# sp-uhh/audio-visual-vad

Hardware: AMD Instinct MI355X
Metric: AV frame-pairs/sec (fwd+bwd) (higher is better)
Workload: dtype f32; 1 GPU; AV_net fused training step (WaveNet-W0 encoder + ResNet-18 trunk + concat + 2xLSTM1024 + FC, masked BCE, backward, RCCL all-reduce, fused Adam): BASELINE configs[3]/[4] per-GPU shard; per_gpu_frame_pairs=1024, global_frame_pairs=1024, sequences_per_gpu=64, parallelism=dp1, reserved_cus=0, reported_block=median

## Files before the change

### audio-visual-vad_amd/csrc/igemm.h

```cpp
#pragma once
#include "common.h"
#include <type_traits>

namespace igemm {

constexpr int BK = 32;

struct NoCtx {};

struct EpiStore {
  static constexpr bool PLAIN = true;
  float* C;
  long ldc;
  const float* bias;
  int mode;
  int cs = 1;
  double* stat = nullptr;
  __device__ __forceinline__ float* ptr(int m, int n) const { return C + (long)m * ldc + (long)n * cs; }
};
template <class Epi, class = void>
struct HasStat : std::false_type {};
template <class Epi>
struct HasStat<Epi, std::void_t<decltype(Epi::stat)>> : std::true_type {};

// ... 308 lines not shown
template <class Epi, class = void>
struct HasFinish : std::false_type {};
template <class Epi>
struct HasFinish<Epi, std::void_t<decltype(&Epi::finish4)>> : std::true_type {};

typedef __bf16 bf16x8 __attribute__((ext_vector_type(8)));
typedef __bf16 bf16x4 __attribute__((ext_vector_type(4)));
typedef float f32x4v __attribute__((ext_vector_type(4)));
constexpr int LDH = 40;

template <class Op, int BX, int NTH>
struct Stage {
  static constexpr int VEC = Op::VEC;
  static constexpr int NV = BX * BK / (NTH * VEC);
  static constexpr int LD = Op::KCONTIG ? BX + 1 : BX + 4;
  static constexpr int NCTX = (Op::KCONTIG || PerVec<Op>::value) ? NV : 1;
  static constexpr int TILE_F32 = BK * LD;
  static constexpr int TILE_BF = BX * LDH / 2;
  __device__ static __forceinline__ void coord(int t, int i, int& xl, int& kl) {
    if (Op::KCONTIG) {
      if (VEC == 4) { kl = (t & 7) * 4; xl = (t >> 3) + (NTH / 8) * i; }
      else { kl = t & 31; xl = (t >> 5) + (NTH / 32) * i; }
    } else {
      if (VEC == 4) { constexpr int Q = BX / 4; xl = (t % Q) * 4; kl = t / Q + (NTH / Q) * i; }
      else { xl = t % BX; kl = t / BX + (NTH / BX) * i; }
    }
  }
  __device__ static __forceinline__ void to_lds(float* S, int t, const float (&st0)[NV][VEC], const Op& op, unsigned okmask) {
    float st[NV][VEC];
#pragma unroll
    for (int i = 0; i < NV; ++i)
#pragma unroll
      for (int j = 0; j < VEC; ++j) {
        float v = st0[i][j];
        if constexpr (HasPost<Op>::value) v = op.post(v);
#ifdef AVVAD_ABL_NOSEL
        st[i][j] = v;
#else
        st[i][j] = ((okmask >> i) & 1u) ? v : 0.f;
#endif
      }
#pragma unroll
    for (int i = 0; i < NV; ++i) {
      int xl, kl;
      coord(t, i, xl, kl);
      if constexpr (Op::KCONTIG) {
#pragma unroll
        for (int j = 0; j < VEC; ++j) S[(kl + j) * LD + xl] = st[i][j];
      } else if constexpr (VEC == 4) {
        *reinterpret_cast<float4*>(S + kl * LD + xl) = make_float4(st[i][0], st[i][1], st[i][2], st[i][3]);
      } else {
        S[kl * LD + xl] = st[i][0];
      }
    }
  }
  __device__ static __forceinline__ void to_lds_bf(__bf16* S, int t, const float (&st0)[NV][VEC], const Op& op, unsigned okmask) {
#pragma unroll
    for (int i = 0; i < NV; ++i) {
      int xl, kl;
      coord(t, i, xl, kl);
      float st[VEC];
#pragma unroll
      for (int j = 0; j < VEC; ++j) {
        float v = st0[i][j];
        if constexpr (HasPost<Op>::value) v = op.post(v);
        st[j] = ((okmask >> i) & 1u) ? v : 0.f;
      }
      if (Op::KCONTIG) {
        if constexpr (VEC == 4) {
          const f32x4v f = {st[0], st[1], st[2], st[3]};
          *reinterpret_cast<bf16x4*>(S + xl * LDH + kl) = __builtin_convertvector(f, bf16x4);
        } else {
          S[xl * LDH + kl] = (__bf16)st[0];
        }
      } else {
#pragma unroll
        for (int j = 0; j < VEC; ++j) S[(xl + j) * LDH + kl] = (__bf16)st[j];
      }
    }
  }
};

template <int BM, int BN, bool DB, int NTH, class AOp, class BOp, class Epi, bool BF = false>
__global__ void __launch_bounds__(NTH, NTH == 512 ? 4 : ((DB || BM * BN < 128 * 128) ? 2 : 3))
    kernel(const AOp A, const BOp B, const Epi E, const int M, const int N, const int flags, const int ktiles,
           const int full_rounds, const int rem_tiles, const int kchunks, float* __restrict__ const slab) {
  const bool stagger = (flags & 1) != 0;
  typedef Stage<AOp, BM, NTH> SA;
  typedef Stage<BOp, BN, NTH> SB;
  constexpr int WGN = (BM == 256) ? 2 : NTH / 128;
  constexpr int WGM = NTH / 64 / WGN;
  constexpr int TM = BM / (32 * WGM), TN = BN / (32 * WGN);
  constexpr int TILE = BF ? SA::TILE_BF + SB::TILE_BF : BK * SA::LD + BK * SB::LD;
  constexpr int AOFF = BF ? SA::TILE_BF : BK * SA::LD;
  const int t_stage = threadIdx.x;
  __shared__ __attribute__((aligned(16))) float smem[(DB ? 2 : 1) * TILE];
  auto stage = [&](float* dst, const float (&ra)[SA::NV][SA::VEC], const float (&rb)[SB::NV][SB::VEC], unsigned ma, unsigned mb) {
    if constexpr (BF) {
      SA::to_lds_bf(reinterpret_cast<__bf16*>(dst), t_stage, ra, A, ma);
      SB::to_lds_bf(reinterpret_cast<__bf16*>(dst + AOFF), t_stage, rb, B, mb);
    } else {
      SA::to_lds(dst, t_stage, ra, A, ma);
      SB::to_lds(dst + AOFF, t_stage, rb, B, mb);
    }
  };

  const int t = threadIdx.x;
  const int lane = t & 63, wave = t >> 6;
  const int li = lane & 31, lh = lane >> 5;
  const int wm = wave / WGN, wn = wave % WGN;
  const int ntn = (N + BN - 1) / BN;

#ifdef AVVAD_PROF
  if (t == 0 && blockIdx.x < 2048) {
    g_prof_blk[2 * blockIdx.x] = __builtin_amdgcn_s_memrealtime();
    g_prof_clk[blockIdx.x] = __builtin_amdgcn_s_memtime();
    g_prof_hw[blockIdx.x] = ((unsigned long long)__builtin_amdgcn_s_getreg((3 << 11) | (0 << 6) | 20) << 32) |
                            (unsigned)__builtin_amdgcn_s_getreg((31 << 11) | (0 << 6) | 4);
  }
#endif
  const long G = gridDim.x;
  const long g = xcd_remap(blockIdx.x, gridDim.x);
  long rem_iters = (long)rem_tiles * ktiles;
  if constexpr (HasSched<Epi>::value) rem_iters = E.sched.total();
  long it = g * rem_iters / G;
  const long it_end = (g + 1) * rem_iters / G;
  const long ntiles_all = (long)((M + BM - 1) / BM) * ntn;
  int round = 0;
  long cell = g;

  for (;;) {
    int tile, kt0, kt1;
    int klen = ktiles;
    if (kchunks > 0) {
      if (cell >= (long)kchunks * ntiles_all) break;
      const int c = (int)(cell / ntiles_all);
      tile = (int)(cell - (long)c * ntiles_all);
      kt0 = (int)((long)c * ktiles / kchunks);
      kt1 = (int)((long)(c + 1) * ktiles / kchunks);
      cell += G;
      if (kt1 <= kt0) continue;
    } else if (round < full_rounds) {
      const long tl = (long)round * G + g;
      ++round;
      if (tl >= ntiles_all) continue;
      tile = (int)tl; kt0 = 0; kt1 = ktiles;
    } else if (it < it_end) {
      if constexpr (HasSched<Epi>::value) {
        E.sched.locate(it, tile, kt0, klen);
      } else {
        const long tr = it / ktiles;
        tile = (int)((long)full_rounds * G + tr);
        kt0 = (int)(it - tr * ktiles);
      }
      kt1 = (int)min((long)klen, kt0 + (it_end - it));
      it += kt1 - kt0;
    } else {
      break;
    }
    const int m0 = (tile / ntn) * BM, n0 = (tile % ntn) * BN;

    typename AOp::Ctx actx[SA::NCTX];
    typename BOp::Ctx bctx[SB::NCTX];
#pragma unroll
    for (int i = 0; i < SA::NCTX; ++i) {
      int xl, kl;
      SA::coord(t, i, xl, kl);
// ... 477 lines not shown

template <int BM, int BN, class AOp, class BOp, class Epi>
static inline int launch(const AOp& a, const BOp& b, const Epi& e_in, int M, int N, int K, int split_k_hint,
                         hipStream_t s, float* slab = nullptr, bool allow_bf16 = true, bool* finished = nullptr) {
  Epi e = e_in;
  if (M <= 0 || N <= 0 || K <= 0) return AVVAD_EINVAL;
  const int ktiles = (K + BK - 1) / BK;
  const long ntiles = (long)cdiv(M, BM) * cdiv(N, BN);
  const long iters = ntiles * ktiles;
  const AvvadTune& tn = avvad_tune();
  const int var = tn.igemm_variant;
  constexpr bool BIG = (BM == 128 && BN == 128);
  constexpr bool TALL = (BM == 256);
  const int variant = TALL ? 3 : (var >= 0 ? var : (BIG ? 2 : 1));
  int per_cu;
  if (variant == 3) per_cu = 2;
  else if (variant == 0) per_cu = BIG ? 2 : (BM * BN >= 128 * 64 ? 3 : 4);
  else if (variant == 1 || !BIG) per_cu = BIG ? 3 : (BM * BN >= 128 * 64 ? 4 : 6);
  else per_cu = 2;
  const int cus = (tn.max_cus > 0 && tn.max_cus < NUM_CU) ? tn.max_cus : NUM_CU;
  long G = (long)cus * per_cu;
  if (G * BM * BN > (long)SLAB_FLOATS) G = (long)(SLAB_FLOATS / ((size_t)BM * BN));
  const bool no_sk = !slab || tn.no_streamk == 1 || tn.no_streamk == 10 + e.mode ||
                     (double)ntiles * ktiles * (double)G >= 4.0e9;
  long full_rounds = ntiles / G, rem = ntiles - full_rounds * G;
  int kchunks = 0;
  if (split_k_hint > 1 && e.mode != 0 && ntiles <= G && tn.kmajor) {
    long best = -1;
    for (int r = 1; r <= 2; ++r) {
      long nc = r * G / ntiles;
      if (nc > ktiles) nc = ktiles;
      if (nc < 1) nc = 1;
      const long rr = (nc * ntiles + G - 1) / G;
      const long cost = rr * ((ktiles + nc - 1) / nc) + rr * 8;
      if (best < 0 || cost < best) { best = cost; kchunks = (int)nc; }
    }
    full_rounds = 0; rem = 0;
    if ((long)kchunks * ntiles < G) G = (long)kchunks * ntiles;
  } else {
    if (no_sk || rem * 10 >= G * 9) {
      if (rem > 0) ++full_rounds;
      rem = 0;
    }
    if (rem > 0 && full_rounds == 0) {
      const long cap = iters / 4 > 0 ? iters / 4 : 1;
      if (G > cap) G = cap;
    }
  }
  const int fr = (int)full_rounds, rt = (int)rem;
  const bool bf = allow_bf16 && tn.bf16;
  bool stat = false;
  if constexpr (std::is_same<Epi, EpiStore>::value) {
    stat = e.stat != nullptr;
    if (stat && (e.cs != 1 || (e.ldc & 3) || (N & 3) || (((uintptr_t)e.C) & 15) || kchunks > 0 || e.bias != nullptr)) return AVVAD_EINVAL;
  }
  if constexpr (HasFinish<Epi>::value) {
    e.active = (rt > 0 && kchunks == 0 && fr == 0 && (long)rt == ntiles) ? 1 : 0;
    if (finished) *finished = e.active != 0;
  } else if (finished) {
    *finished = false;
  }
  const int kflags = tn.stagger ? 1 : 0;
#define AVVAD_IGEMM_LAUNCH(DBV, NTHV)                                                                                       \
  do {                                                                                                                      \
    if (bf)                                                                                                                 \
      hipLaunchKernelGGL((kernel<BM, BN, DBV, NTHV, AOp, BOp, Epi, true>), dim3((int)G), dim3(NTHV), 0, s, a, b, e, M, N, kflags, \
                         ktiles, fr, rt, kchunks, slab);                                                                    \
    else                                                                                                                    \
      hipLaunchKernelGGL((kernel<BM, BN, DBV, NTHV, AOp, BOp, Epi, false>), dim3((int)G), dim3(NTHV), 0, s, a, b, e, M, N, kflags, \
                         ktiles, fr, rt, kchunks, slab);                                                                    \
  } while (0)
  if constexpr (TALL) {
    AVVAD_IGEMM_LAUNCH(false, 512);
  } else {
    if (variant == 0) AVVAD_IGEMM_LAUNCH(true, 256);
    else if (variant == 1 || !BIG) AVVAD_IGEMM_LAUNCH(false, 256);
    else AVVAD_IGEMM_LAUNCH(true, (BIG ? 512 : 256));
  }
#undef AVVAD_IGEMM_LAUNCH
  if (rt > 0 && kchunks == 0 && stat) {
    if constexpr (std::is_same<Epi, EpiStore>::value)
      hipLaunchKernelGGL((fixup_tile<BM, BN>), dim3(rt), dim3(256), 0, s, e, slab, M, N, ktiles, G, fr, rt, cdiv(N, BN));
  } else if (rt > 0 && kchunks == 0) {
    const int deep = tn.no_fixup1 > 1 ? tn.no_fixup1 : 6;
    if ((G + rt - 1) / rt <= deep && tn.no_fixup1 != 1)
      hipLaunchKernelGGL((fixup1<BM, BN, Epi>), dim3(rt * (BM * BN / 1024)), dim3(256), 0, s, e, slab, M, N, ktiles, G, fr, rt, cdiv(N, BN));
    else
      hipLaunchKernelGGL((fixup<BM, BN, Epi>), dim3(rt * (BM * BN / 256)), dim3(256), 0, s, e, slab, M, N, ktiles, G, fr, rt, cdiv(N, BN));
  }
  AVVAD_LAUNCH_CHECK();
  return AVVAD_OK;
}

template <class AOp, class BOp, class Epi>
static inline int launch_cls(const AOp& a, const BOp& b, const Epi& e, int Mp, int N, hipStream_t s, float* slab) {
  constexpr int BM = 128, BN = 128;
  if (Mp <= 0 || N <= 0 || !slab) return AVVAD_EINVAL;
  const AvvadTune& tn = avvad_tune();
  const long ntiles = (long)cdiv(Mp, BM) * cdiv(N, BN);
  const int cus = (tn.max_cus > 0 && tn.max_cus < NUM_CU) ? tn.max_cus : NUM_CU;
  long G = (long)cus * 2;
  if (G * BM * BN > (long)SLAB_FLOATS) G = (long)(SLAB_FLOATS / ((size_t)BM * BN));
  const long R = e.sched.total();
  if (R <= 0 || (double)R * (double)G >= 4.0e9) return AVVAD_EINVAL;
  if (G > R / 4) G = R / 4 > 0 ? R / 4 : 1;
  bool stat = false;
  if constexpr (HasStat<Epi>::value) {
    stat = e.stat != nullptr;
    if (stat && (e.cs != 1 || (e.ldc & 3) || (N & 3) || (((uintptr_t)e.C) & 15) || (e.W & 3))) return AVVAD_EINVAL;
  }
  hipLaunchKernelGGL((kernel<BM, BN, true, 512, AOp, BOp, Epi, false>), dim3((int)G), dim3(512), 0, s, a, b, e, Mp, N,
                     tn.stagger ? 1 : 0, 1, 0, (int)ntiles, 0, slab);
  if (stat) {
    if constexpr (HasStat<Epi>::value)
      hipLaunchKernelGGL((fixup_tile<BM, BN, Epi>), dim3((int)ntiles), dim3(256), 0, s, e, slab, Mp, N, 1, G, 0, (int)ntiles, cdiv(N, BN));
  } else if ((G + ntiles - 1) / ntiles <= 6) {
    hipLaunchKernelGGL((fixup1<BM, BN, Epi>), dim3((int)ntiles * (BM * BN / 1024)), dim3(256), 0, s, e, slab, Mp, N, 1, G, 0,
                       (int)ntiles, cdiv(N, BN));
  } else {
    hipLaunchKernelGGL((fixup<BM, BN, Epi>), dim3((int)ntiles * (BM * BN / 256)), dim3(256), 0, s, e, slab, Mp, N, 1, G, 0, (int)ntiles,
                       cdiv(N, BN));
  }
  AVVAD_LAUNCH_CHECK();
  return AVVAD_OK;
}

}
```

### audio-visual-vad_amd/csrc/trunk.hip

```cpp
#include "bgemm.h"
#include "conv64.h"

using convop::Geom;

namespace {

#include "bn_kernels.h"

constexpr int NCONV = AVVAD_TRUNK_NCONV;

struct ConvSpec {
  int cin, cout, ks, stride, pad;
  int stage;
  int role;
};

struct Plan {
  int N, H, W;
  int h[6], w[6];
  ConvSpec conv[NCONV];
  Geom geom[NCONV];
  size_t wf[NCONV], wd[NCONV];
  size_t wf16[NCONV], wd16[NCONV];
  size_t bn_scale, bn_shift, bn_mean, bn_invstd;
// ... 392 lines not shown
      const int r = i / W, c = i - r * W;
      img[(r + 3) * LDW + c + 3] = xn[i];
    }
    __syncthreads();
    const __amdgpu_buffer_rsrc_t rdy = brsrc(dy + (long)n * Ho * Wo * 64, Ho * Wo * 64 * 4);
    constexpr int RB = 4;
    float b0[RB][STEM_WH], b1[RB][STEM_WH];
    auto rowload = [&](int ho0, float (&b)[RB][STEM_WH]) {
#pragma unroll
      for (int rr = 0; rr < RB; ++rr)
#pragma unroll
        for (int sw = 0; sw < STEM_WH; ++sw)
          b[rr][sw] = bload(rdy, (sw < wh && ho0 + rr < Ho) ? voff : BUF_OOB, ((ho0 + rr) * Wo + 2 * sw) * 256);
    };
    auto rowmul = [&](int ho0, const float (&b)[RB][STEM_WH]) {
#pragma unroll
      for (int rr = 0; rr < RB; ++rr) {
        if (ho0 + rr >= Ho) break;
        const float* ap = img + abase + 2 * (ho0 + rr) * LDW;
#pragma unroll
        for (int sw = 0; sw < STEM_WH; ++sw)
          if (sw < wh) acc = mfma32(ap[4 * sw], b[rr][sw], acc);
      }
    };
    rowload(0, b0);
    for (int ho = 0; ho < Ho; ho += 2 * RB) {
      if (ho + RB < Ho) rowload(ho + RB, b1);
      __builtin_amdgcn_sched_barrier(0);
      rowmul(ho, b0);
      if (ho + RB >= Ho) break;
      if (ho + 2 * RB < Ho) rowload(ho + 2 * RB, b0);
      __builtin_amdgcn_sched_barrier(0);
      rowmul(ho + RB, b1);
    }
  }
  float* out = slab + (long)blockIdx.x * (49 * 64);
#pragma unroll
  for (int r = 0; r < 16; ++r) {
    const int t = mt * 32 + mfma32_row(r, lh);
    if (t < 49) out[t * 64 + nt * 32 + li] = acc[r];
  }
}
__global__ void __launch_bounds__(256) stem_wgrad_reduce(const float* __restrict__ slab, int nslab, float* __restrict__ pk) {
  __shared__ float sm[8][32];
  const int el = threadIdx.x & 31, grp = threadIdx.x >> 5;
  const int i = blockIdx.x * 32 + el;
  float s = 0.f;
#pragma unroll 4
  for (int b = grp; b < nslab; b += 8) s += slab[(long)b * (49 * 64) + i];
  sm[grp][el] = s;
  __syncthreads();
  if (grp != 0) return;
#pragma unroll
  for (int k = 1; k < 8; ++k) s += sm[k][el];
  pk[i] = s;
}

static inline bool fits_u30(long n) { return n >= 0 && n < (1L << 30); }
static inline bool taps_fit(const Geom& g) { return g.KS * g.KS <= 32; }
static inline bool fits_buf(long n_floats) { return n_floats >= 0 && n_floats < (1L << 29) - 64; }
static inline bool stem_kernel_ok(const Geom& g) {
  const int LDW = (g.W + 6) | 1;
  return g.C == 1 && g.KS == 7 && g.stride == 2 && g.pad == 3 && g.Co == 64 && (size_t)(g.H + 6) * LDW * sizeof(float) <= 48 * 1024 &&
         !avvad_tune().no_stem_kernel;
}
static inline bool stem_wgrad_ok(const Geom& g, bool slab) {
  return stem_kernel_ok(g) && (g.Wo & 1) == 0 && g.Wo <= 2 * STEM_WH && slab && (long)g.Ho * g.Wo * 64 * 4 < (1L << 31);
}
static inline long cls_tile_cap() {
  if (avvad_tune().cls_cap > 0) return avvad_tune().cls_cap;
  return 4L * ((avvad_tune().max_cus > 0 && avvad_tune().max_cus < 256) ? avvad_tune().max_cus : 256);
}
static inline bool cls_common(const Geom& g, bool slab) {
  return avvad_tune().bf16 == 0 && !avvad_tune().no_cls && slab && g.KS == 3 && g.pad == 1 && g.N >= 128 && g.C % 32 == 0 &&
         g.Co % 32 == 0 && g.Ho >= 2 && g.Wo >= 2 && avvad_tune().igemm_variant < 0 && !avvad_tune().no_buf &&
         avvad_tune().no_streamk == 0;
}
static inline bool conv_fwd_cls_ok(const Geom& g, bool slab) {
  if (!cls_common(g, slab) || g.Co % 4 || g.Co < 128) return false;
  const long tiles = (long)g.Ho * g.Wo * cdiv(g.N, 128) * cdiv(g.Co, 128);
  return tiles <= cls_tile_cap() &&
         fits_buf((long)g.N * g.H * g.W * g.C) && fits_buf(9L * g.C * g.Co);
}
static inline bool conv_dgrad_cls_ok(const Geom& g, bool slab) {
  if (!cls_common(g, slab) || (g.stride != 1 && (g.stride != 2 || avvad_tune().no_s2_cls)) || g.C % 4 || g.C < 128) return false;
  const long tiles = (long)g.H * g.W * cdiv(g.N, 128) * cdiv(g.C, 128);
  return tiles <= cls_tile_cap() &&
         fits_buf((long)g.N * g.Ho * g.Wo * g.Co) && fits_buf(9L * g.C * g.Co);
}
static inline bool conv_wgrad_tap_ok(const Geom& g, bool slab) {
  if (!cls_common(g, slab) || g.C % 128 || g.Co % 4 || g.Co < 128) return false;
  return 9L * (g.C / 128) * cdiv(g.Co, 128) <= cls_tile_cap() &&
         fits_buf((long)g.N * g.H * g.W * g.C) && fits_buf((long)g.N * g.Ho * g.Wo * g.Co);
}
static inline int conv64_cus() { return (avvad_tune().max_cus > 0 && avvad_tune().max_cus < 256) ? avvad_tune().max_cus : 256; }
static inline bool conv64_ok(const Geom& g, bool b16) {
  const long M = (long)g.N * g.H * g.W;
  return (b16 || avvad_tune().bf16 == 0) && !avvad_tune().no_conv64 && g.C == 64 && g.Co == 64 && g.KS == 3 && g.stride == 1 &&
         g.pad == 1 && g.Ho == g.H && g.Wo == g.W && M > 0 && fits_buf(M * 64) &&
         (unsigned long)(M + 64) * (unsigned long)(g.H * g.W) < 0x100000000ull;
}
static inline bool conv64_wgrad_ok(const Geom& g, bool slab) {
  return conv64_ok(g, false) && slab && g.W <= conv64::WG_MAXW && (size_t)conv64_cus() * conv64::WG_PART <= igemm::SLAB_FLOATS &&
         (long)g.N * g.H * g.W * 256 < (1L << 31);
}

static inline bool native_bf16() { return avvad_tune().bf16 == 1; }
static inline bool bf16_conv_ok(const Geom& g) {
  return g.C % 64 == 0 && g.Co % 64 == 0 && taps_fit(g) && fits_buf((long)g.N * g.H * g.W * g.C / 2) &&
         fits_buf((long)g.N * g.Ho * g.Wo * g.Co / 2) && fits_buf((long)g.KS * g.KS * g.C * g.Co / 2);
}
static inline bool cls16_common(const Geom& g, bool slab) {
  return !avvad_tune().no_cls && slab && g.KS == 3 && g.pad == 1 && g.N >= 128 && g.Ho >= 2 && g.Wo >= 2 && g.Ho * g.Wo <= 9 &&
         avvad_tune().no_streamk == 0;
}
static inline bool conv_fwd16_cls_ok(const Geom& g, bool slab) {
  if (!cls16_common(g, slab) || g.Co < 128) return false;
  return (long)g.Ho * g.Wo * cdiv(g.N, 128) * cdiv(g.Co, 128) <= cls_tile_cap();
}
static inline bool conv_dgrad16_cls_ok(const Geom& g, bool slab) {
  const bool form = g.stride == 1 ? cls16_common(g, slab)
                                  : g.stride == 2 && g.KS == 3 && g.pad == 1 && !avvad_tune().no_cls && !avvad_tune().no_s2_cls &&
                                        avvad_tune().no_streamk == 0 && slab && g.N >= 128;
  return form && g.C >= 128 && (long)g.H * g.W * cdiv(g.N, 128) * cdiv(g.C, 128) <= cls_tile_cap();
}
static inline bool conv_wgrad16_tap_ok(const Geom& g, bool slab) {
  return cls16_common(g, slab) && g.C % 128 == 0 && g.Co >= 128 && 9L * (g.C / 128) * cdiv(g.Co, 128) <= cls_tile_cap();
}

enum Form { STEM, CONV64, CLS, TAP, PARITY, ENGINE };
struct ConvForm {
  Form form;
  int rows, cols;
  bool buf;
  int chunks;
};
static ConvForm fwd_form(const Geom& g, bool b16, bool slab) {
  const long M = (long)g.N * g.Ho * g.Wo;
  const int cols = g.Co <= 64 ? 64 : 128;
  if (conv64_ok(g, b16)) return {CONV64, 0, 0, false, conv64::grid_for((long)g.N * g.H * g.W, conv64_cus())};
  if (b16 ? conv_fwd16_cls_ok(g, slab) : conv_fwd_cls_ok(g, slab)) return {CLS, 0, 0, false, g.Ho * g.Wo * cdiv(g.N, 128)};
  if (b16) return {ENGINE, 128, cols, true, cdiv(M, 128)};
  if (g.C == 1) return stem_kernel_ok(g) ? ConvForm{STEM, 0, 0, false, g.N} : ConvForm{ENGINE, 128, 64, false, 0};
  const int rows = g.Co <= 64 && !avvad_tune().no_tall ? 256 : 128;
  const bool buf = fits_buf((long)g.N * g.H * g.W * g.C) && fits_buf((long)g.KS * g.KS * g.C * g.Co) && !avvad_tune().no_buf;
  return {ENGINE, rows, cols, buf, cdiv(M, rows)};
}
static ConvForm dgrad_form(const Geom& g, bool b16, bool slab) {
  if (conv64_ok(g, b16)) return {CONV64};
  if (b16 ? conv_dgrad16_cls_ok(g, slab) : conv_dgrad_cls_ok(g, slab)) return {CLS};
  const int cols = g.C <= 64 ? 64 : 128;
  const bool buf = b16 || (fits_buf((long)g.N * g.Ho * g.Wo * g.Co) && fits_buf((long)g.KS * g.KS * g.C * g.Co) && !avvad_tune().no_buf);
  if (g.stride == 2) return {PARITY, 128, cols, buf};
  return {ENGINE, cols == 64 && !b16 && !avvad_tune().no_tall ? 256 : 128, cols, buf};
}
static ConvForm wgrad_form(const Geom& g, bool b16, bool slab) {
  const int cols = g.Co <= 64 ? 64 : 128;
  if (b16) return conv_wgrad16_tap_ok(g, slab) ? ConvForm{TAP} : ConvForm{ENGINE, 128, cols, true};
  if (conv64_wgrad_ok(g, slab)) return {CONV64};
  if (conv_wgrad_tap_ok(g, slab)) return {TAP};
  if (g.C == 1) return stem_wgrad_ok(g, slab) ? ConvForm{STEM} : ConvForm{ENGINE, 64, 64, false};
  const bool buf = fits_buf((long)g.N * g.H * g.W * g.C) && fits_buf((long)g.N * g.Ho * g.Wo * g.Co) && !avvad_tune().no_buf;
  return {ENGINE, 128, cols, buf};
}

static igemm::ClassSched fwd_sched(const Geom& g, int kc) {
  const int lsh = ((g.Ho - 1) * g.stride - g.pad + 2 > g.H - 1) ? 1 : 0, lsw = ((g.Wo - 1) * g.stride - g.pad + 2 > g.W - 1) ? 1 : 0;
  return igemm::ClassSched{g.Ho, g.Wo, cdiv(g.Co, 128), g.C / kc, cdiv(g.N, 128), 3, 1, lsh, 1, lsw};
}
static igemm::ClassSched dgrad_sched(const Geom& g, int kc) {
  igemm::ClassSched sc{g.H, g.W, cdiv(g.C, 128), g.Co / kc, cdiv(g.N, 128), 3, 1, 1, 1, 1};
  if (g.stride == 2) { sc.s2 = 1; sc.Hq = g.Ho; sc.Wq = g.Wo; }
  return sc;
}
template <class Gemm>
static int dgrad_parity(float* dx, const Geom& g, int accumulate, hipStream_t s, Gemm gemm) {
  const long n = (long)g.N * g.H * g.W * g.C;
  if (!accumulate) hipLaunchKernelGGL(zero_f32, dim3(ew_grid(n)), dim3(256), 0, s, dx, n);
  for (int ph = 0; ph < 2; ++ph)
    for (int pw = 0; pw < 2; ++pw) {
      convop::S2Class c;
      c.ph = ph; c.pw = pw;
      c.Hc = (g.H - ph + 1) / 2; c.Wc = (g.W - pw + 1) / 2;
      c.kh0 = (ph + g.pad) & 1; c.kw0 = (pw + g.pad) & 1;
      c.nkh = c.kh0 < g.KS ? (g.KS - c.kh0 + 1) / 2 : 0;
      c.nkw = c.kw0 < g.KS ? (g.KS - c.kw0 + 1) / 2 : 0;
      c.oh = (ph + g.pad - c.kh0) / 2; c.ow = (pw + g.pad - c.kw0) / 2;
      const int Mc = g.N * c.Hc * c.Wc, ntap = c.nkh * c.nkw;
      if (Mc <= 0 || ntap <= 0) continue;
      if (ntap > 4) return AVVAD_EINVAL;
      c.mg_ntap = convop::div_magic(ntap); c.mg_nkw = convop::div_magic(c.nkw);
      const convop::EpiS2 e{dx, g.C, nullptr, 1, 1, g.H, g.W, c.Hc, c.Wc, ph, pw, convop::div_magic(c.Hc * c.Wc), convop::div_magic(c.Wc)};
      if ((unsigned long)(Mc + 128) * (unsigned long)(c.Hc * c.Wc) >= 0x100000000ull) return AVVAD_EINVAL;
      if (const int rc = gemm(c, Mc, ntap, e)) return rc;
    }
  return AVVAD_OK;
}

static int conv64_launch(bool b16, bool flip, const float* x, const float* wpk, float* y, const Geom& g, int accumulate, hipStream_t s,
                         double* stat) {
  const int M = g.N * g.H * g.W;
  const int grid = conv64::grid_for(M, conv64_cus());
  const unsigned mg_hw = convop::div_magic((unsigned)(g.H * g.W)), mg_w = convop::div_magic((unsigned)g.W);
  auto k = b16 ? (flip ? conv64::kernel16<true> : conv64::kernel16<false>) : (flip ? conv64::kernel<true> : conv64::kernel<false>);
  hipLaunchKernelGGL(k, dim3(grid), dim3(conv64::NW * 64), 0, s, x, wpk, y, M, g.H, g.W, mg_hw, mg_w, accumulate, stat);
  AVVAD_LAUNCH_CHECK();
  return AVVAD_OK;
}
static int conv_fwd_cls(const float* x, const float* wf, float* y, const Geom& g, hipStream_t s, float* slab, double* stat) {
  const int MB = cdiv(g.N, 128), P = g.Ho * g.Wo;
  const igemm::ClassSched sc = fwd_sched(g, 32);
  const igemm::ClassRow cr{P, convop::div_magic(P)};
  convop::Im2colFwdCls a{x, g, g.N, cr, sc};
  convop::ColTapRowsCls b{wf, g.Co, g.Co, g.C, 3, 0, cr, sc};
  igemm::EpiCls e{y, (long)P * g.Co, nullptr, 0};
  e.stat = stat; e.W = g.Co; e.rows = g.N; e.cr = cr; e.sched = sc;
  return igemm::launch_cls(a, b, e, MB * P * 128, g.Co, s, slab);
}
static int conv_dgrad_cls(const float* dy, const float* wd, float* dx, const Geom& g, int accumulate, hipStream_t s, float* slab) {
  const int MB = cdiv(g.N, 128), P = g.H * g.W;
  const igemm::ClassSched sc = dgrad_sched(g, 32);
  const igemm::ClassRow cr{P, convop::div_magic(P)};
  convop::Im2colDgradCls a{dy, g, g.N, cr, sc};
  convop::ColTapRowsCls b{wd, g.C, g.C, g.Co, 3, 1, cr, sc};
  igemm::EpiCls e{dx, (long)P * g.C, nullptr, accumulate ? 1 : 0};
  e.W = g.C; e.rows = g.N; e.cr = cr; e.sched = sc;
  return igemm::launch_cls(a, b, e, MB * P * 128, g.C, s, slab);
}

template <bool BUF>
static int conv_fwd_t(const float* x, const float* wf, float* y, const Geom& g, const ConvForm& f, hipStream_t s, float* slab, double* stat) {
  const int M = g.N * g.Ho * g.Wo, K = g.KS * g.KS * g.C;
  igemm::EpiStore e{y, g.Co, nullptr, 0};
  if (g.C == 1) {
    igemm::ColPlain<4> b{wf, g.Co, g.Co, K, 0};
    convop::StemFwd a{x, g, M, K};
    return igemm::launch<128, 64>(a, b, e, M, g.Co, K, 1, s, slab);
  }
  e.stat = stat;
  if (g.C % 32 || g.Co % 4 || !taps_fit(g)) return AVVAD_EINVAL;
  if (!fits_u30((long)g.N * g.H * g.W * g.C) || !fits_u30((long)K * g.Co)) return AVVAD_EINVAL;
  const int T = g.KS * g.KS;
  convop::ColTapRows<BUF> b{wf, g.Co, g.Co, K, g.C, T, convop::div_magic(T)};
  convop::Im2colFwd<BUF> a{x, g, M, convop::tap_div(T, g.KS)};
  if (f.rows == 256) return igemm::launch<256, 64>(a, b, e, M, g.Co, K, 1, s, slab);
  if (f.cols == 64) return igemm::launch<128, 64>(a, b, e, M, g.Co, K, 1, s, slab);
  return igemm::launch<128, 128>(a, b, e, M, g.Co, K, 1, s, slab);
}
static int conv_fwd(const float* x, const float* wf, float* y, const Geom& g, hipStream_t s, float* slab, double* stat = nullptr) {
  const ConvForm f = fwd_form(g, false, slab);
  switch (f.form) {
    case STEM: {
      const int LDW = (g.W + 6) | 1;
      hipLaunchKernelGGL(stem_fwd_mfma, dim3(g.N), dim3(256), (size_t)(g.H + 6) * LDW * sizeof(float), s, x, wf, y, g.H, g.W, g.Ho, g.Wo,
                         LDW, stat);
      AVVAD_LAUNCH_CHECK();
      return AVVAD_OK;
    }
    case CONV64: return conv64_launch(false, false, x, wf, y, g, 0, s, stat);
    case CLS: return conv_fwd_cls(x, wf, y, g, s, slab, stat);
    default: return f.buf ? conv_fwd_t<true>(x, wf, y, g, f, s, slab, stat) : conv_fwd_t<false>(x, wf, y, g, f, s, slab, stat);
  }
}
template <bool BUF>
static int conv_dgrad_t(const float* dy, const float* wd, float* dx, const Geom& g, const ConvForm& f, int accumulate, hipStream_t s,
                        float* slab) {
  const int M = g.N * g.H * g.W, K = g.KS * g.KS * g.Co;
  if (g.Co % 32 || g.C % 4 || !taps_fit(g)) return AVVAD_EINVAL;
  if (!fits_u30((long)g.N * g.Ho * g.Wo * g.Co) || !fits_u30((long)K * g.C)) return AVVAD_EINVAL;
  if (f.form == PARITY)
    return dgrad_parity(dx, g, accumulate, s, [&](const convop::S2Class& c, int Mc, int ntap, const convop::EpiS2& e) {
      convop::Im2colDgradS2<BUF> a{dy, g, c, Mc};
      convop::ColSegRows<BUF> b{wd, g.C, g.C, ntap * g.Co, ntap, {0, 0, 0, 0}, convop::div_magic(ntap)};
      for (int ia = 0; ia < c.nkh; ++ia)
        for (int ib = 0; ib < c.nkw; ++ib) b.rowbase[ia * c.nkw + ib] = ((c.kh0 + 2 * ia) * g.KS + (c.kw0 + 2 * ib)) * g.Co;
      return f.cols == 64 ? igemm::launch<128, 64>(a, b, e, Mc, g.C, ntap * g.Co, 1, s, slab)
                          : igemm::launch<128, 128>(a, b, e, Mc, g.C, ntap * g.Co, 1, s, slab);
    });
  igemm::EpiStore e{dx, g.C, nullptr, accumulate ? 1 : 0};
  const int T = g.KS * g.KS;
  convop::ColTapRows<BUF> b{wd, g.C, g.C, K, g.Co, T, convop::div_magic(T)};
  convop::Im2colDgrad<BUF> a{dy, g, M, convop::tap_div(T, g.KS)};
  if (f.rows == 256) return igemm::launch<256, 64>(a, b, e, M, g.C, K, 1, s, slab);
  if (f.cols == 64) return igemm::launch<128, 64>(a, b, e, M, g.C, K, 1, s, slab);
  return igemm::launch<128, 128>(a, b, e, M, g.C, K, 1, s, slab);
}
static int conv_dgrad(const float* dy, const float* wd, float* dx, const Geom& g, int accumulate, hipStream_t s, float* slab) {
  const ConvForm f = dgrad_form(g, false, slab);
  switch (f.form) {
    case CONV64: return conv64_launch(false, true, dy, wd, dx, g, accumulate, s, nullptr);
    case CLS: return conv_dgrad_cls(dy, wd, dx, g, accumulate, s, slab);
    default: return f.buf ? conv_dgrad_t<true>(dy, wd, dx, g, f, accumulate, s, slab) : conv_dgrad_t<false>(dy, wd, dx, g, f, accumulate, s, slab);
  }
}
template <bool BUF>
static int conv_wgrad_t(const float* x, const float* dy, float* pk, const Geom& g, const ConvForm& f, hipStream_t s, float* slab) {
  const int M = g.KS * g.KS * g.C, K = g.N * g.Ho * g.Wo;
  igemm::ColPlain<4, BUF> b{dy, g.Co, g.Co, K, 0};
  const int ktiles = cdiv(K, igemm::BK);
  if (g.C == 1) {
    igemm::EpiStore e{pk, g.Co, nullptr, 0};
    convop::StemWgradX a{x, g, M, K};
    int split = 1024; if (split > ktiles) split = ktiles;
    return igemm::launch<64, 64>(a, b, e, M, g.Co, K, split, s, slab);
  }
  if (g.C % 32) return AVVAD_EINVAL;
  convop::EpiWgrad e{pk, g.Co, nullptr, 0, 1, g.C, g.KS * g.KS, convop::div_magic(g.KS * g.KS)};
  if ((unsigned long)(K + igemm::BK) * (unsigned long)(g.Ho * g.Wo) >= 0x100000000ull) return AVVAD_EINVAL;
  if (!fits_u30((long)g.N * g.H * g.W * g.C) || !fits_u30((long)K * g.Co)) return AVVAD_EINVAL;
  convop::WgradX<BUF> a{x, g, M, K, convop::div_magic(g.Ho * g.Wo), convop::div_magic(g.Wo)};
  const int nb = cdiv(M, 128) * cdiv(g.Co, f.cols);
  int split = cdiv(1024, nb); if (split > ktiles) split = ktiles;
  if (f.cols == 64) return igemm::launch<128, 64>(a, b, e, M, g.Co, K, split, s, slab);
  return igemm::launch<128, 128>(a, b, e, M, g.Co, K, split, s, slab);
}
static inline igemm::TapSched tap_sched(const Geom& g, int tiles_per_tap) {
  const int NP = cdiv(g.N, 128) * 128;
  const int lsh = ((g.Ho - 1) * g.stride - g.pad + 2 > g.H - 1) ? 1 : 0, lsw = ((g.Wo - 1) * g.stride - g.pad + 2 > g.W - 1) ? 1 : 0;
  return igemm::TapSched{g.Ho, g.Wo, tiles_per_tap, NP / 32, 3, 1, lsh, 1, lsw};
}
static int conv_wgrad_tap(const float* x, const float* dy, float* pk, const Geom& g, hipStream_t s, float* slab) {
  const int M = 9 * g.C;
  const igemm::TapSched sc = tap_sched(g, (g.C / 128) * cdiv(g.Co, 128));
  convop::WgradXTap a{x, g, M, g.C, g.N, convop::div_magic(g.C), sc};
  convop::ColDyTap b{dy, g, g.Co, g.C, g.N, sc};
  igemm::EpiTap e{pk, g.Co, nullptr, 0};
  e.Mrows = M; e.sched = sc;
  return igemm::launch_cls(a, b, e, M, g.Co, s, slab);
}
static int conv64_wgrad(const float* x, const float* dy, float* pk, const Geom& g, hipStream_t s, float* slab) {
  const int NR = g.N * g.H;
  const int grid = NR < conv64_cus() ? NR : conv64_cus();
  hipLaunchKernelGGL(conv64::wgrad_kernel, dim3(grid), dim3(conv64::WG_WAVES * 64), 0, s, x, dy, slab, NR, g.H, g.W,
                     convop::div_magic((unsigned)g.H));
  hipLaunchKernelGGL(conv64::wgrad_reduce, dim3(conv64::WG_PART / 256), dim3(256), 0, s, (const float*)slab, grid, pk);
  AVVAD_LAUNCH_CHECK();
  return AVVAD_OK;
}
static int conv_wgrad(const float* x, const float* dy, float* pk, const Geom& g, hipStream_t s, float* slab) {
  const ConvForm f = wgrad_form(g, false, slab);
  switch (f.form) {
    case STEM: {
      const int LDW = (g.W + 6) | 1;
      const int nb = g.N < 256 ? g.N : 256;
      hipLaunchKernelGGL(stem_wgrad_mfma, dim3(nb), dim3(256), (size_t)(g.H + 6) * LDW * sizeof(float), s, x, dy, slab, g.N, g.H, g.W,
                         g.Ho, g.Wo, LDW);
      hipLaunchKernelGGL(stem_wgrad_reduce, dim3(49 * 64 / 32), dim3(256), 0, s, slab, nb, pk);
      AVVAD_LAUNCH_CHECK();
      return AVVAD_OK;
    }
    case CONV64: return conv64_wgrad(x, dy, pk, g, s, slab);
    case TAP: return conv_wgrad_tap(x, dy, pk, g, s, slab);
    default: return f.buf ? conv_wgrad_t<true>(x, dy, pk, g, f, s, slab) : conv_wgrad_t<false>(x, dy, pk, g, f, s, slab);
  }
// ... 309 lines not shown
                       ws + p.p0, am, d->N, p.h[1], p.w[1], p.h[2], p.w[2]);
  }
  auto cfwd = [&](const float* xin, int i, float* yout) -> int {
    if (b16) return conv_fwd16(xin, ws + p.wf16[i], yout, p.geom[i], s, ws + p.slab, fused_stat(&p, ws, i, d));
    return conv_fwd(xin, ws + p.wf[i], yout, p.geom[i], s, ws + p.slab, fused_stat(&p, ws, i, d));
  };
  auto act = b16 ? bn_act<true, false> : bn_act<false, false>;
  auto act_id = b16 ? bn_act<true, true> : bn_act<false, false>;
  const float* x = ws + p.p0;
  int ci = 1;
  const int widths[4] = {64, 128, 256, 512};
  for (int st = 0; st < 4; ++st)
    for (int b = 0; b < 2; ++b) {
      const int C = widths[st];
      const size_t* o = p.blk[st * 2 + b];
      const bool ds = (b == 0 && st > 0);
      const long M = N * p.h[st + 2] * p.w[st + 2];
      const long nq = M * C / 4;
      const int i1 = ci, i2 = ci + 1, id = ci + 2;
      unsigned char* qmo = d->save_for_backward ? reinterpret_cast<unsigned char*>(ws + p.qm[st * 2 + b]) : (unsigned char*)nullptr;
      if ((rc = cfwd(x, i1, ws + o[0]))) return rc;
      if ((rc = bn_prepare(&p, ws, i1, ws + o[0], M, prm, d, s))) return rc;
      hipLaunchKernelGGL(act, dim3(ew_grid(nq)), dim3(256), 0, s, ws + o[0], ws + p.bn_scale + i1 * MAXC, ws + p.bn_shift + i1 * MAXC,
                         (const float*)nullptr, (const float*)nullptr, (const float*)nullptr, ws + o[1], nq, C, 1, (unsigned char*)nullptr);
      if ((rc = cfwd(ws + o[1], i2, ws + o[2]))) return rc;
      if ((rc = bn_prepare(&p, ws, i2, ws + o[2], M, prm, d, s))) return rc;
      if (ds) {
        if ((rc = cfwd(x, id, ws + o[3]))) return rc;
        if ((rc = bn_prepare(&p, ws, id, ws + o[3], M, prm, d, s))) return rc;
        hipLaunchKernelGGL(act, dim3(ew_grid(nq)), dim3(256), 0, s, ws + o[2], ws + p.bn_scale + i2 * MAXC, ws + p.bn_shift + i2 * MAXC,
                           ws + o[3], ws + p.bn_scale + id * MAXC, ws + p.bn_shift + id * MAXC, ws + o[4], nq, C, 1, qmo);
      } else {
        hipLaunchKernelGGL(act_id, dim3(ew_grid(nq)), dim3(256), 0, s, ws + o[2], ws + p.bn_scale + i2 * MAXC, ws + p.bn_shift + i2 * MAXC,
                           x, (const float*)nullptr, (const float*)nullptr, ws + o[4], nq, C, 1, qmo);
      }
      x = ws + o[4];
      ci += ds ? 3 : 2;
    }
  auto avg = b16 ? avgpool_fwd<true> : avgpool_fwd<false>;
  hipLaunchKernelGGL(avg, dim3(ew_grid(N * 512)), dim3(256), 0, s, x, feat, d->N, p.h[5] * p.w[5], 512);
  AVVAD_LAUNCH_CHECK();
  return AVVAD_OK;
}

extern "C" int avvad_trunk_bwd(const float* frames, const avvad_trunk_params* prm, const float* dfeat,
                               const avvad_trunk_grads* g, const avvad_trunk_desc* d, void* wsv, size_t ws_bytes,
                               avvad_stream_t sv) {
  AVVAD_ENTER();
  BwdCuCap cu_cap;
  if (!frames || !prm || !dfeat || !g || !d || !wsv || ws_misaligned(wsv) || !d->save_for_backward) return AVVAD_EINVAL;
  hipStream_t s = (hipStream_t)sv;
  Plan p;
  make_plan(d, &p);
  if (ws_bytes < p.total * sizeof(float)) return AVVAD_EWORKSPACE;
  float* ws = (float*)wsv;
  int rc;
  const long N = d->N;
  float* G0 = ws + p.G[0];
  float* G1 = ws + p.G[1];
  float* G2 = ws + p.G[2];
  float* G3 = ws + p.G[3];
  hipLaunchKernelGGL(avgpool_bwd, dim3(ew_grid(N * p.h[5] * p.w[5] * 512)), dim3(256), 0, s, dfeat, G0, d->N,
                     p.h[5] * p.w[5], 512);
  const bool b16 = native_bf16();
  auto wgrad = [&](int i, const float* xin, const float* dyraw) -> int {
    if (!g->conv_w[i]) return AVVAD_OK;
    if (b16 && i > 0) return conv_wgrad16(xin, dyraw, ws + p.wg[i], p.geom[i], s, ws + p.slab);
    return conv_wgrad(xin, dyraw, ws + p.wg[i], p.geom[i], s, ws + p.slab);
  };
  auto dgrad = [&](const float* dyv, int i, float* dxv, int accumulate) -> int {
    if (b16) return conv_dgrad16(dyv, ws + p.wd16[i], dxv, p.geom[i], accumulate, s, ws + p.slab);
    return conv_dgrad(dyv, ws + p.wd[i], dxv, p.geom[i], accumulate, s, ws + p.slab);
  };
  int ci = NCONV;
  for (int st = 3; st >= 0; --st)
    for (int b = 1; b >= 0; --b) {
      const bool ds = (b == 0 && st > 0);
      ci -= ds ? 3 : 2;
      const int i1 = ci, i2 = ci + 1, id = ci + 2;
      const size_t* o = p.blk[st * 2 + b];
      const float* x = (st == 0 && b == 0) ? ws + p.p0 : (b == 1 ? ws + p.blk[st * 2][4] : ws + p.blk[st * 2 - 1][4]);
      const long M = N * p.h[st + 2] * p.w[st + 2];
      const unsigned char* qmb = reinterpret_cast<const unsigned char*>(ws + p.qm[st * 2 + b]);
      if (ds) {
        if ((rc = bn_backward(&p, ws, i2, ws + o[2], G0, ws + o[4], G1, nullptr, M, prm, g, d, s, false, qmb, b16))) return rc;
        if ((rc = bn_backward(&p, ws, id, ws + o[3], G0, ws + o[4], G2, nullptr, M, prm, g, d, s, false, qmb, b16))) return rc;
        if ((rc = wgrad(id, x, G2))) return rc;
        if ((rc = dgrad(G2, id, G3, 0))) return rc;
      } else {
        if ((rc = bn_backward(&p, ws, i2, ws + o[2], G0, ws + o[4], G1, G3, M, prm, g, d, s, false, qmb, b16))) return rc;
      }
      if ((rc = wgrad(i2, ws + o[1], G1))) return rc;
      if ((rc = dgrad(G1, i2, G2, 0))) return rc;
      if ((rc = bn_backward(&p, ws, i1, ws + o[0], G2, ws + o[1], G1, nullptr, M, prm, g, d, s, true, nullptr, b16))) return rc;
      if ((rc = wgrad(i1, x, G1))) return rc;
      if ((rc = dgrad(G1, i1, G3, 1))) return rc;
      float* t = G0; G0 = G3; G3 = t;
    }
  if (g->conv_w[0] || g->bn_w[0] || g->bn_b[0]) {
    float* g0 = ws + p.g0;
    const bool fuse0 = !avvad_tune().no_fused_stats;
    int grid0 = ew_grid(N * p.h[1] * p.w[1] * 16);
    if (fuse0 && grid0 > 2048) grid0 = 2048;
    hipLaunchKernelGGL(stem_pool_relu_bwd, dim3(grid0), dim3(256), 0, s, ws + p.c0,
                       ws + p.bn_scale, ws + p.bn_shift, reinterpret_cast<const unsigned*>(ws + p.am), G0, g0, d->N, p.h[1], p.w[1],
                       p.h[2], p.w[2], fuse0 ? ws + p.bn_mean : (const float*)nullptr, fuse0 ? ws + p.bn_invstd : (const float*)nullptr,
                       fuse0 ? reinterpret_cast<double*>(ws + p.part) : (double*)nullptr);
    const long M0 = N * p.h[1] * p.w[1];
    if ((rc = bn_backward(&p, ws, 0, ws + p.c0, g0, nullptr, g0, nullptr, M0, prm, g, d, s, false, nullptr, false, fuse0 ? grid0 : 0))) return rc;
    if ((rc = wgrad(0, frames, g0))) return rc;
  }
  {
    UnpackTab tab;
    int nb = 0;
    bool any = false;
    for (int i = 0; i < NCONV; ++i) {
      const ConvSpec& c = p.conv[i];
      const bool done = g->conv_w[i] && (i > 0 || g->conv_w[0]);
      tab.pk[i] = ws + p.wg[i];
      tab.dw[i] = done ? g->conv_w[i] : (float*)nullptr;
      tab.cout[i] = c.cout; tab.cin[i] = c.cin; tab.ks[i] = c.ks;
      tab.blk0[i] = nb;
      nb += i == 0 ? cdiv(64 * 3 * 49, 256) : (c.cout / 32) * (c.cin / 32);
      any = any || done;
    }
    tab.blk0[NCONV] = nb;
    if (any) hipLaunchKernelGGL(unpack_all, dim3(nb), dim3(256), 0, s, tab);
  }
  AVVAD_LAUNCH_CHECK();
  return AVVAD_OK;
}
```

Measured before the change: 60170 frame-pairs/s.

## Extend class-split dgrad to 64-column tiles and streamline trunk backward dgrad

```diff
diff --git a/audio-visual-vad_amd/csrc/igemm.h b/audio-visual-vad_amd/csrc/igemm.h
--- a/audio-visual-vad_amd/csrc/igemm.h
+++ b/audio-visual-vad_amd/csrc/igemm.h
@@ -414,7 +414,7 @@
 };
 
 template <int BM, int BN, bool DB, int NTH, class AOp, class BOp, class Epi, bool BF = false>
-__global__ void __launch_bounds__(NTH, NTH == 512 ? 4 : ((DB || BM * BN < 128 * 128) ? 2 : 3))
+__global__ void __launch_bounds__(NTH, (NTH == 512 || HasSched<Epi>::value) ? 4 : ((DB || BM * BN < 128 * 128) ? 2 : 3))
     kernel(const AOp A, const BOp B, const Epi E, const int M, const int N, const int flags, const int ktiles,
            const int full_rounds, const int rem_tiles, const int kchunks, float* __restrict__ const slab) {
   const bool stagger = (flags & 1) != 0;
@@ -1058,6 +1058,11 @@
     if constexpr (std::is_same<Epi, EpiStore>::value)
       hipLaunchKernelGGL((fixup_tile<BM, BN>), dim3(rt), dim3(256), 0, s, e, slab, M, N, ktiles, G, fr, rt, cdiv(N, BN));
   } else if (rt > 0 && kchunks == 0) {
+    const long pool = (long)rt * ktiles;
+    if (!HasFinish<Epi>::value && pool % G == 0 && (pool / G) % ktiles == 0) {
+      AVVAD_LAUNCH_CHECK();
+      return AVVAD_OK;
+    }
     const int deep = tn.no_fixup1 > 1 ? tn.no_fixup1 : 6;
     if ((G + rt - 1) / rt <= deep && tn.no_fixup1 != 1)
       hipLaunchKernelGGL((fixup1<BM, BN, Epi>), dim3(rt * (BM * BN / 1024)), dim3(256), 0, s, e, slab, M, N, ktiles, G, fr, rt, cdiv(N, BN));
@@ -1068,14 +1073,17 @@
   return AVVAD_OK;
 }
 
-template <class AOp, class BOp, class Epi>
+template <int BN = 128, class AOp, class BOp, class Epi>
 static inline int launch_cls(const AOp& a, const BOp& b, const Epi& e, int Mp, int N, hipStream_t s, float* slab) {
-  constexpr int BM = 128, BN = 128;
+  static_assert(BN == 128 || BN == 64, "column tile of a position-class product");
+  constexpr int BM = 128;
+  constexpr bool WIDE = BN == 128;
+  constexpr int NTH = WIDE ? 512 : 256;
   if (Mp <= 0 || N <= 0 || !slab) return AVVAD_EINVAL;
   const AvvadTune& tn = avvad_tune();
   const long ntiles = (long)cdiv(Mp, BM) * cdiv(N, BN);
   const int cus = (tn.max_cus > 0 && tn.max_cus < NUM_CU) ? tn.max_cus : NUM_CU;
-  long G = (long)cus * 2;
+  long G = (long)cus * (WIDE ? 2 : 4);
   if (G * BM * BN > (long)SLAB_FLOATS) G = (long)(SLAB_FLOATS / ((size_t)BM * BN));
   const long R = e.sched.total();
   if (R <= 0 || (double)R * (double)G >= 4.0e9) return AVVAD_EINVAL;
@@ -1085,7 +1093,7 @@
     stat = e.stat != nullptr;
     if (stat && (e.cs != 1 || (e.ldc & 3) || (N & 3) || (((uintptr_t)e.C) & 15) || (e.W & 3))) return AVVAD_EINVAL;
   }
-  hipLaunchKernelGGL((kernel<BM, BN, true, 512, AOp, BOp, Epi, false>), dim3((int)G), dim3(512), 0, s, a, b, e, Mp, N,
+  hipLaunchKernelGGL((kernel<BM, BN, WIDE, NTH, AOp, BOp, Epi, false>), dim3((int)G), dim3(NTH), 0, s, a, b, e, Mp, N,
                      tn.stagger ? 1 : 0, 1, 0, (int)ntiles, 0, slab);
   if (stat) {
     if constexpr (HasStat<Epi>::value)
diff --git a/audio-visual-vad_amd/csrc/trunk.hip b/audio-visual-vad_amd/csrc/trunk.hip
--- a/audio-visual-vad_amd/csrc/trunk.hip
+++ b/audio-visual-vad_amd/csrc/trunk.hip
@@ -498,10 +498,16 @@
   return tiles <= cls_tile_cap() &&
          fits_buf((long)g.N * g.H * g.W * g.C) && fits_buf(9L * g.C * g.Co);
 }
+static inline long cls64_s2_tile_cap() {
+  return 64L * ((avvad_tune().max_cus > 0 && avvad_tune().max_cus < 256) ? avvad_tune().max_cus : 256);
+}
+static inline int dgrad_cls_cols(const Geom& g) { return g.C == 64 ? 64 : 128; }
 static inline bool conv_dgrad_cls_ok(const Geom& g, bool slab) {
-  if (!cls_common(g, slab) || (g.stride != 1 && (g.stride != 2 || avvad_tune().no_s2_cls)) || g.C % 4 || g.C < 128) return false;
-  const long tiles = (long)g.H * g.W * cdiv(g.N, 128) * cdiv(g.C, 128);
-  return tiles <= cls_tile_cap() &&
+  const bool s2 = g.stride == 2 && !avvad_tune().no_s2_cls;
+  if (!cls_common(g, slab) || (g.stride != 1 && !s2) || g.C % 4 || (g.C < 128 && !(s2 && g.C == 64))) return false;
+  const int cols = dgrad_cls_cols(g);
+  const long tiles = (long)g.H * g.W * cdiv(g.N, 128) * cdiv(g.C, cols);
+  return tiles <= (cols == 64 ? cls64_s2_tile_cap() : cls_tile_cap()) &&
          fits_buf((long)g.N * g.Ho * g.Wo * g.Co) && fits_buf(9L * g.C * g.Co);
 }
 static inline bool conv_wgrad_tap_ok(const Geom& g, bool slab) {
@@ -584,8 +590,8 @@
   const int lsh = ((g.Ho - 1) * g.stride - g.pad + 2 > g.H - 1) ? 1 : 0, lsw = ((g.Wo - 1) * g.stride - g.pad + 2 > g.W - 1) ? 1 : 0;
   return igemm::ClassSched{g.Ho, g.Wo, cdiv(g.Co, 128), g.C / kc, cdiv(g.N, 128), 3, 1, lsh, 1, lsw};
 }
-static igemm::ClassSched dgrad_sched(const Geom& g, int kc) {
-  igemm::ClassSched sc{g.H, g.W, cdiv(g.C, 128), g.Co / kc, cdiv(g.N, 128), 3, 1, 1, 1, 1};
+static igemm::ClassSched dgrad_sched(const Geom& g, int kc, int cols = 128) {
+  igemm::ClassSched sc{g.H, g.W, cdiv(g.C, cols), g.Co / kc, cdiv(g.N, 128), 3, 1, 1, 1, 1};
   if (g.stride == 2) { sc.s2 = 1; sc.Hq = g.Ho; sc.Wq = g.Wo; }
   return sc;
 }
@@ -635,12 +641,14 @@
 }
 static int conv_dgrad_cls(const float* dy, const float* wd, float* dx, const Geom& g, int accumulate, hipStream_t s, float* slab) {
   const int MB = cdiv(g.N, 128), P = g.H * g.W;
-  const igemm::ClassSched sc = dgrad_sched(g, 32);
+  const int cols = dgrad_cls_cols(g);
+  const igemm::ClassSched sc = dgrad_sched(g, 32, cols);
   const igemm::ClassRow cr{P, convop::div_magic(P)};
   convop::Im2colDgradCls a{dy, g, g.N, cr, sc};
   convop::ColTapRowsCls b{wd, g.C, g.C, g.Co, 3, 1, cr, sc};
   igemm::EpiCls e{dx, (long)P * g.C, nullptr, accumulate ? 1 : 0};
   e.W = g.C; e.rows = g.N; e.cr = cr; e.sched = sc;
+  if (cols == 64) return igemm::launch_cls<64>(a, b, e, MB * P * 128, g.C, s, slab);
   return igemm::launch_cls(a, b, e, MB * P * 128, g.C, s, slab);
 }
 
@@ -686,6 +694,14 @@
   if (!fits_u30((long)g.N * g.Ho * g.Wo * g.Co) || !fits_u30((long)K * g.C)) return AVVAD_EINVAL;
   if (f.form == PARITY)
     return dgrad_parity(dx, g, accumulate, s, [&](const convop::S2Class& c, int Mc, int ntap, const convop::EpiS2& e) {
+      if constexpr (BUF) {
+        if (g.KS == 1 && g.pad == 0 && c.Hc == g.Ho && c.Wc == g.Wo && (((uintptr_t)dy | (uintptr_t)wd) & 15) == 0) {
+          igemm::RowVec4 a{dy, g.Co, Mc, g.Co, 0};
+          igemm::ColPlain<4, true> b{wd, g.C, g.C, g.Co, 0};
+          return f.cols == 64 ? igemm::launch<128, 64>(a, b, e, Mc, g.C, g.Co, 1, s, slab)
+                              : igemm::launch<128, 128>(a, b, e, Mc, g.C, g.Co, 1, s, slab);
+        }
+      }
       convop::Im2colDgradS2<BUF> a{dy, g, c, Mc};
       convop::ColSegRows<BUF> b{wd, g.C, g.C, ntap * g.Co, ntap, {0, 0, 0, 0}, convop::div_magic(ntap)};
       for (int ia = 0; ia < c.nkh; ++ia)
@@ -1161,19 +1177,21 @@
       const float* x = (st == 0 && b == 0) ? ws + p.p0 : (b == 1 ? ws + p.blk[st * 2][4] : ws + p.blk[st * 2 - 1][4]);
       const long M = N * p.h[st + 2] * p.w[st + 2];
       const unsigned char* qmb = reinterpret_cast<const unsigned char*>(ws + p.qm[st * 2 + b]);
+      float* Ga = G2;
       if (ds) {
         if ((rc = bn_backward(&p, ws, i2, ws + o[2], G0, ws + o[4], G1, nullptr, M, prm, g, d, s, false, qmb, b16))) return rc;
         if ((rc = bn_backward(&p, ws, id, ws + o[3], G0, ws + o[4], G2, nullptr, M, prm, g, d, s, false, qmb, b16))) return rc;
         if ((rc = wgrad(id, x, G2))) return rc;
-        if ((rc = dgrad(G2, id, G3, 0))) return rc;
+        Ga = G0;
       } else {
         if ((rc = bn_backward(&p, ws, i2, ws + o[2], G0, ws + o[4], G1, G3, M, prm, g, d, s, false, qmb, b16))) return rc;
       }
       if ((rc = wgrad(i2, ws + o[1], G1))) return rc;
-      if ((rc = dgrad(G1, i2, G2, 0))) return rc;
-      if ((rc = bn_backward(&p, ws, i1, ws + o[0], G2, ws + o[1], G1, nullptr, M, prm, g, d, s, true, nullptr, b16))) return rc;
+      if ((rc = dgrad(G1, i2, Ga, 0))) return rc;
+      if ((rc = bn_backward(&p, ws, i1, ws + o[0], Ga, ws + o[1], G1, nullptr, M, prm, g, d, s, true, nullptr, b16))) return rc;
       if ((rc = wgrad(i1, x, G1))) return rc;
-      if ((rc = dgrad(G1, i1, G3, 1))) return rc;
+      if ((rc = dgrad(G1, i1, G3, ds ? 0 : 1))) return rc;
+      if (ds && (rc = dgrad(G2, id, G3, 1))) return rc;
       float* t = G0; G0 = G3; G3 = t;
     }
   if (g->conv_w[0] || g->bn_w[0] || g->bn_b[0]) {
```

After: 60550 frame-pairs/s, median of 6. No clear change (+0.6%).
